# tatary/ramses

Hardware: AMD Instinct MI355X
Metric: cell-updates/s (Godunov sweep), uniform Sedov3D (higher is better)
Workload: dtype f64

## Files before the change

ramses_amd/csrc/hydro_sweep.hip:

```cpp
#include <hip/hip_runtime.h>

#include <type_traits>

#include "difmag_core.hpp"
#include "hydro_core.hpp"
#include "sweep_args.hpp"

namespace ramses_amd {

#ifdef RAMSES_AMD_FAST
#define SWEEP_NS fastmode
#else
#define SWEEP_NS strictmode
#endif

namespace SWEEP_NS {

constexpr int BX = 64;
#ifndef TILE_SWEEP_BY
#define TILE_SWEEP_BY 12
#endif

template <int BY, int NV>
struct Plane {
  double v[NV][BY][BX];
};

template <int ST, int BY, int NV, bool MASK, bool GRAV, int NX = 0, bool DUTY = false, bool R3 = false, int DPN = 0>
struct Lds {
  static constexpr int NF = NV + NX;
  static constexpr int RING = (ST == 3 || R3) ? 3 : 2;
#ifndef SWEEP_PARK_PLAIN
#ifdef RAMSES_AMD_FAST
#define SWEEP_PARK_PLAIN 1
#else
#define SWEEP_PARK_PLAIN 0
#endif
#endif
  static constexpr bool PARK = MASK || ((GRAV || SWEEP_PARK_PLAIN) && BY == 12);
  static constexpr int MR = PARK ? BY - 2 : BY;
  static constexpr int M0 = PARK ? 1 : 0;
  static constexpr size_t q_off = 0;
  static constexpr size_t m_off = q_off + RING * sizeof(Plane<BY, NV>);
  static constexpr size_t park_off = m_off + 2 * sizeof(Plane<MR, NF>);
  static constexpr size_t duty_off = park_off + (PARK ? sizeof(double) * 2 * NF * (BY - 4) * BX : 0);
  static constexpr size_t mask_off = duty_off + (DUTY ? sizeof(double) * 2 * NF * BX : 0);
  static constexpr size_t sloc_off = mask_off + (MASK ? 3 * BY * BX : 0);
  static constexpr size_t dpark_off = sloc_off + (MASK ? 4 * BY * BX : 0);
  static constexpr size_t bytes = dpark_off + sizeof(double) * DPN * (BY - 4) * BX;
};
template <int RS, int NV>
constexpr int dif_parked() { return (NV == 5 && RS == RIEMANN_EXACT) ? 2 * NV + 2 : ((NV == 6) ? NV + 2 : 0); }

__device__ __forceinline__ double wave_shr1(double v) {
  int lo = __double2loint(v), hi = __double2hiint(v);
  lo = __builtin_amdgcn_update_dpp(lo, lo, 0x138, 0xf, 0xf, false);
  hi = __builtin_amdgcn_update_dpp(hi, hi, 0x138, 0xf, 0xf, false);
  return __hiloint2double(hi, lo);
}
template <bool TIED = false>
__device__ __forceinline__ double wave_shl1(double v) {
  int lo = __double2loint(v), hi = __double2hiint(v);
  lo = TIED ? __builtin_amdgcn_update_dpp(lo, lo, 0x130, 0xf, 0xf, false) : __builtin_amdgcn_update_dpp(0, lo, 0x130, 0xf, 0xf, true);
  hi = TIED ? __builtin_amdgcn_update_dpp(hi, hi, 0x130, 0xf, 0xf, false) : __builtin_amdgcn_update_dpp(0, hi, 0x130, 0xf, 0xf, true);
  return __hiloint2double(hi, lo);
}

enum { ROLE_HALO = 0, ROLE_LOW = 1, ROLE_HIGH = 2, ROLE_FULL = 3, ROLE_HALO_HI = 4, ROLE_FULL_LO = 5 };

#ifndef SWEEP_YDUTY
#define SWEEP_YDUTY 0
#endif
template <int ST, int RS, int BY, bool GRAV, int SCHEME, int NV, bool MASK, int NE = 0, bool PFIX = false>
constexpr bool y_duty() {
  return SWEEP_YDUTY && SWEEP_PARK_PLAIN && RS == RIEMANN_LLF && BY == 12 && ST != 3 && !GRAV && SCHEME == 0 && NV == 5 && !MASK && NE == 0 && !PFIX;
}
template <int BY, bool DUTY>
constexpr int yflux_wave(int f) { return !DUTY ? f : (f == 2 ? 0 : (f == BY - 2 ? BY - 1 : f)); }

#ifndef SWEEP_TRIM
#ifdef RAMSES_AMD_FAST
#define SWEEP_TRIM 1
#else
#define SWEEP_TRIM 0
#endif
#endif

#ifndef SWEEP_CYCLE_PROBE
#define SWEEP_CYCLE_PROBE 0
#endif
#if SWEEP_CYCLE_PROBE
constexpr int PROBE_BLOCKS = 8192, PROBE_ROWS = 12, PROBE_WORDS = 6;
static __device__ unsigned long long sweep_cycle_probe[PROBE_BLOCKS][PROBE_ROWS][PROBE_WORDS];
#endif

typedef unsigned int v2u32 __attribute__((ext_vector_type(2)));
constexpr unsigned BUF_RANGE = 0x7fffffffu;
constexpr unsigned BUF_OOB = 0xffffffffu;
#ifndef SWEEP_STORE_AUX
#define SWEEP_STORE_AUX 0
#endif
__device__ __forceinline__ double plane_load(const double *var_base, unsigned plane_bytes, unsigned off) {
  __amdgpu_buffer_rsrc_t r = __builtin_amdgcn_make_buffer_rsrc(const_cast<double *>(var_base), 0, BUF_RANGE, 0x00020000);
  return __builtin_bit_cast(double, __builtin_amdgcn_raw_buffer_load_b64(r, off, plane_bytes, 0));
}
__device__ __forceinline__ void plane_store(double *var_base, unsigned plane_bytes, unsigned off, double x) {
  __amdgpu_buffer_rsrc_t r = __builtin_amdgcn_make_buffer_rsrc(var_base, 0, BUF_RANGE, 0x00020000);
  __builtin_amdgcn_raw_buffer_store_b64(__builtin_bit_cast(v2u32, x), r, off, plane_bytes, SWEEP_STORE_AUX);
}

__device__ __forceinline__ int wave_shr1_i(int v) { return __builtin_amdgcn_update_dpp(v, v, 0x138, 0xf, 0xf, false); }
__device__ __forceinline__ int wave_shl1_i(int v) { return __builtin_amdgcn_update_dpp(0, v, 0x130, 0xf, 0xf, true); }
__device__ __forceinline__ int stat_load(const unsigned char *base, unsigned ncell, unsigned lane_cell, unsigned plane_cell) {
  __amdgpu_buffer_rsrc_t r = __builtin_amdgcn_make_buffer_rsrc(const_cast<unsigned char *>(base), 0, ncell, 0x00020000);
  return (int)__builtin_amdgcn_raw_buffer_load_b8(r, lane_cell, plane_cell, 0);
}
__device__ __forceinline__ int dir_load(const int *base, unsigned plane_ints, unsigned col) {
  __amdgpu_buffer_rsrc_t r = __builtin_amdgcn_make_buffer_rsrc(const_cast<int *>(base), 0, BUF_RANGE, 0x00020000);
  return (int)__builtin_amdgcn_raw_buffer_load_b32(r, col * 4u, plane_ints * 4u, 0);
}

template <int NV>
__device__ __forceinline__ void load_uold_cell(const double *uold, long pitch_var, unsigned odd_var, unsigned pb, unsigned off, double (&u)[NV]) {
#pragma unroll
  for (int n = 0; n < NV; n++) u[n] = plane_load(uold + (long)(n & ~1) * pitch_var, pb + (n & 1) * odd_var, off);
}
__device__ __forceinline__ unsigned tile_base_ym(int par, bool inB, unsigned a0, unsigned a1, unsigned b0, unsigned b1) {
  const unsigned a = par ? a1 : a0, b = par ? b1 : b0;
  return inB ? b : a;
}
template <int ST, int RS, int BY, bool GRAV, int SCHEME, int NV, int ROLE, bool MASK, int NE = 0, bool PFIX = false, bool DIFMAG = false>
__device__ __forceinline__ void sweep_march(const SweepArgs &A, unsigned char *smem_raw, const SweepPfix &X = SweepPfix(),
                                            const SweepDifmag &D = SweepDifmag()) {
  static_assert(!PFIX || (MASK && NE == 0 && SCHEME == 0), "pressure_fix: the sweep of a level in tiles, muscl");
  static_assert(!DIFMAG || (MASK && NE == 0 && SCHEME == 0 && !PFIX), "difmag: the sweep of a level in tiles, muscl, no pressure_fix");
  constexpr int NF = NV + (PFIX ? 2 : 0);
  const bool DXPOW2 = A.pow2 != 0;
  constexpr bool DUTY = y_duty<ST, RS, BY, GRAV, SCHEME, NV, MASK, NE, PFIX>();
  static_assert(DUTY || ROLE != ROLE_FULL_LO, "row 2 is a full row like the others unless the y fluxes are shared out");
  constexpr int DPN = DIFMAG ? dif_parked<RS, NV>() : 0;
  typedef Lds<ST, BY, NV, MASK, GRAV, NF - NV, DUTY, DIFMAG, DPN> L;
  double (*dpark)[BY - 4][BX] = reinterpret_cast<double (*)[BY - 4][BX]>(smem_raw + L::dpark_off);
  constexpr int RING = L::RING;
  constexpr bool PARK = L::PARK;
  constexpr int M0 = L::M0;
  Plane<BY, NV> *qring = reinterpret_cast<Plane<BY, NV> *>(smem_raw + L::q_off);
  Plane<L::MR, NF> *mring = reinterpret_cast<Plane<L::MR, NF> *>(smem_raw + L::m_off);
  double (*park)[BY - 4][BX] = reinterpret_cast<double (*)[BY - 4][BX]>(smem_raw + L::park_off);
  double (*yduty)[NF][BX] = reinterpret_cast<double (*)[NF][BX]>(smem_raw + L::duty_off);

  const int tx = threadIdx.x, ty = threadIdx.y;
  const HydroConst &P = A.P;

  const int hb = blockIdx.x;
  int bi = 0;
#pragma unroll
  for (int i = 1; i < 6; i++)
    if (i < A.nbox && hb >= A.box[i].first) bi = i;
  const SweepBox &B = A.box[bi];
  int lb = hb - B.first;
  {
    const int nxcd = 8;
    const int cnt = (bi + 1 < A.nbox ? A.box[bi + 1].first : (int)gridDim.x) - B.first;
    if (cnt % nxcd == 0) {
      const int per = cnt / nxcd;
      lb = (lb % nxcd) * per + lb / nxcd;
    }
  }
#ifndef SWEEP_TILE_YFAST
#define SWEEP_TILE_YFAST 0
#endif
#if SWEEP_TILE_YFAST
  const int tiy = B.ty0 + lb % B.nty;
  const int tix = B.tx0 + (lb / B.nty) % B.ntx;
#else
  const int tix = B.tx0 + lb % B.ntx;
  const int tiy = B.ty0 + (lb / B.ntx) % B.nty;
#endif
  const int tiz = lb / (B.ntx * B.nty);
  int x0 = tix * (BX - 4);
  int y0 = tiy * (BY - 4);
  int z0 = B.zlo + tiz * B.zchunk;
  int z1 = min(z0 + B.zchunk, B.zhi);
  if (MASK) {
    const int4 w = reinterpret_cast<const int4 *>(A.work)[hb];
    x0 = w.x; y0 = w.y; z0 = w.z; z1 = w.w;
  }

  const int xu = x0 - 2 + tx;
  const int yu = y0 - 2 + ty;
  int xi, yi;
  if (A.ng == 0) {
    xi = xu < 0 ? xu + A.nx : (xu >= A.nx ? xu - A.nx : xu);
    xi = xi >= A.nx ? xi % A.nx : xi;
    yi = yu < 0 ? yu + A.ny : (yu >= A.ny ? yu - A.ny : yu);
    yi = yi >= A.ny ? yi % A.ny : yi;
  } else {
    xi = min(max(xu, -A.ng), A.nx + A.ng - 1) + A.ng;
    yi = min(max(yu, -A.ng), A.ny + A.ng - 1) + A.ng;
  }
  const unsigned colb = (unsigned)(xi + yi * (int)A.pitch_y) * 8u;
  int tyu = 0, yis = 0, xa = 0, tA = 0, tB = 0, drow = 0;
  bool inB = false;
  unsigned *sloc = reinterpret_cast<unsigned *>(smem_raw + L::sloc_off);
  if (MASK) {
    tyu = __builtin_amdgcn_readfirstlane(ty);
    const int ys = y0 - 2 + tyu;
    yis = ys < 0 ? ys + A.ny : (ys >= A.ny ? ys - A.ny : ys);
    const int xs = x0 - 2;
    xa = xs < 0 ? xs + A.nx : xs;
    tA = xa >> 6; tB = tA + 1 < A.ntx ? tA + 1 : 0;
    inB = (xa & 63) + tx >= 64;
    drow = A.ntx * (yis >> 3);
    const int lind = (xi & 1) + 2 * (yis & 1);
    sloc[ty * BX + tx] = ((unsigned)((long)lind * A.ngd) + (unsigned)(((xi >> 1) & (TILE_OX - 1)) + TILE_OX * ((yis >> 1) & (TILE_OY - 1)))) * 8u;
  }
  const double *__restrict__ uold = A.uold;
  double *__restrict__ unew = A.unew;
  const double *__restrict__ grav = A.grav;

#ifndef SWEEP_LATE_BASE
#define SWEEP_LATE_BASE 0
#endif
  constexpr bool LATE = SWEEP_LATE_BASE && NV == 5;
#ifndef SWEEP_KEEP_PLAIN
#define SWEEP_KEEP_PLAIN 1
#endif
#ifndef SWEEP_KEEP_STRICT
#define SWEEP_KEEP_STRICT 0
#endif
#if defined(RAMSES_AMD_FAST) || SWEEP_KEEP_STRICT
#ifndef SWEEP_KEEP_LLF_ONLY
#define SWEEP_KEEP_LLF_ONLY 0
#endif
#ifndef SWEEP_KEEP_NOT_HLLC
#define SWEEP_KEEP_NOT_HLLC 1
#endif
  constexpr bool KEEP = (MASK || (SWEEP_KEEP_PLAIN && BY == 12)) && NV == 5 && !LATE && (!SWEEP_KEEP_LLF_ONLY || RS == RIEMANN_LLF) &&
                        (!SWEEP_KEEP_NOT_HLLC || RS != RIEMANN_HLLC);
#else
  constexpr bool KEEP = false;
#endif
  constexpr bool r_fxz = ROLE == ROLE_FULL || ROLE == ROLE_FULL_LO;
  constexpr bool r_trace = ROLE == ROLE_LOW || ROLE == ROLE_HIGH || r_fxz;
  constexpr bool y_give = DUTY && (ROLE == ROLE_FULL_LO || ROLE == ROLE_HIGH);
  constexpr bool y_take = DUTY && (ROLE == ROLE_HALO || ROLE == ROLE_HALO_HI);
  constexpr int DUTY_F = ROLE == ROLE_HALO ? 2 : BY - 2;
  static_assert(!DUTY || (yflux_wave<BY, DUTY>(2) == 0 && yflux_wave<BY, DUTY>(BY - 2) == BY - 1 && yflux_wave<BY, DUTY>(3) == 3),
                "the roles below implement this table");
  constexpr bool TRIM = SWEEP_TRIM != 0 && RS == RIEMANN_LLF && SCHEME == 0 && NE == 0 && !PFIX;
  const bool r_upd = r_fxz && (tx >= 2) && (tx <= BX - 3) && (xu < A.nx) && (yu < A.ny);
  const unsigned colb_upd = r_upd ? colb : BUF_OOB;

  const double dtdx = A.dt / A.dx;
  const double dtxhalf = A.dt * 0.5;

  auto plane_off = [&](int p) -> unsigned {
    int pz;
    if (A.ng == 0) { pz = p < 0 ? p + A.nz : (p >= A.nz ? p - A.nz : p); }
    else { pz = p + A.ng; }
    return (unsigned)pz * (unsigned)(A.pitch_z * 8);
  };
  auto wrap_z = [&](int p) -> int { return p < 0 ? p + A.nz : (p >= A.nz ? p - A.nz : p); };
  constexpr unsigned TILE_VOID = 0x80000000u;
  unsigned sA0 = TILE_VOID, sA1 = TILE_VOID, sB0 = TILE_VOID, sB1 = TILE_VOID;
  unsigned mA0 = TILE_VOID, mA1 = TILE_VOID, mB0 = TILE_VOID, mB1 = TILE_VOID;
  int drow_m = 0;
  if constexpr (DIFMAG) {
    const int ym = yis > 0 ? yis - 1 : A.ny - 1;
    drow_m = A.ntx * (ym >> 3);
  }
  auto tile_of_plane = [&](int p) -> int { return wrap_z(p) >> 3; };
  auto tile_set = [&](int tz) {
    typedef const int __attribute__((address_space(4))) *cdir_p;
    const cdir_p row = (cdir_p)(A.dir + (long)tz * (A.ntx * A.nty) + drow);
    const int ra = row[tA], rb = row[tB];
    const unsigned a = ra < 0 ? TILE_VOID : (unsigned)ra * 8u, b = rb < 0 ? TILE_VOID : (unsigned)rb * 8u;
    if (tz & 1) { sA1 = a; sB1 = b; } else { sA0 = a; sB0 = b; }
    if constexpr (DIFMAG) {
      const cdir_p rowm = (cdir_p)(A.dir + (long)tz * (A.ntx * A.nty) + drow_m);
      const int qa = rowm[tA], qb = rowm[tB];
      const unsigned am = qa < 0 ? TILE_VOID : (unsigned)qa * 8u, bm = qb < 0 ? TILE_VOID : (unsigned)qb * 8u;
      if (tz & 1) { mA1 = am; mB1 = bm; } else { mA0 = am; mB0 = bm; }
    }
  };
  auto zpart = [&](int p) -> unsigned {
    const int pz = wrap_z(p);
    return (unsigned)((long)(pz & 1) * 4 * A.ngd) + (unsigned)(TILE_OX * TILE_OY * ((pz >> 1) & (TILE_OZ - 1)));
  };
  auto tbp = [&](int p) -> unsigned {
    const int par = tile_of_plane(p) & 1;
    const unsigned a = par ? sA1 : sA0, b = par ? sB1 : sB0;
    return (inB ? b : a) + sloc[ty * BX + tx];
  };
  const unsigned odd_var = (unsigned)(A.pitch_var * 8);
  auto load_u = [&](int p, double (&u)[NV]) {
    const unsigned pb = MASK ? zpart(p) * 8u : plane_off(p), off = MASK ? tbp(p) : colb;
#pragma unroll
    for (int n = 0; n < NV; n++)
      u[n] = MASK ? plane_load(uold + (long)(n & ~1) * A.pitch_var, pb + (n & 1) * odd_var, off) : plane_load(uold + (long)n * A.pitch_var, pb, off);
  };
  const double *__restrict__ bsrc = A.base_uold ? uold : unew;
  auto load_base = [&](int p, double (&u)[NF]) {
    const unsigned pb = zpart(p) * 8u, off = tbp(p);
#pragma unroll
    for (int n = 0; n < NV; n++) u[n] = plane_load(bsrc + (long)(n & ~1) * A.pitch_var, pb + (n & 1) * odd_var, off);
    if constexpr (PFIX) { u[NV] = plane_load(X.divu, pb, off); u[NV + 1] = plane_load(X.enew, pb, off); }
  };
  double dif_cy = 0.0;
  double dif_c0 = 0.0, dif_c1 = 0.0;
  int ok_zlo = 0;
  int spre = 0;
  unsigned char *smask = smem_raw + L::mask_off;
  auto load_g = [&](int p, double (&g)[3]) {
    if (GRAV) {
      const unsigned pb = MASK ? zpart(p) * 8u : plane_off(p), off = MASK ? tbp(p) : colb;
#pragma unroll
      for (int d = 0; d < 3; d++) g[d] = plane_load(grav + (long)d * A.pitch_var, pb, off);
    } else {
      g[0] = g[1] = g[2] = 0.0;
    }
  };

  double qmz[NV];
  double fzlo[NF];
  double upre[NV], gpre[3];
  double rold = 0.0, sold[NV > 5 ? NV - 5 : 1];
  double ukeep[NV];
#pragma unroll
  for (int n = 0; n < NV; n++) ukeep[n] = 0.0;

  double rinv_c = 0.0;
#if SWEEP_CYCLE_PROBE
  unsigned long long pr_a = 0, pr_w = 0, pr_b = 0, pr_n = 0;
#endif

  int sa = 0, sb = 1, sc = 2;

  if (MASK) {
    const int t0 = tile_of_plane(z0 - 2), t1 = t0 + 1 < A.ntz ? t0 + 1 : 0;
    tile_set(t0);
    tile_set(t1);
    __syncthreads();
    if (r_trace) spre = stat_load(A.stat, (unsigned)A.pitch_var, tbp(z0 - 1) >> 3, zpart(z0 - 1));
  }
  {
    double u[NV], g[3], q[NV];
    load_u(z0 - 2, u); load_g(z0 - 2, g);
    ctoprim_cell<NV, GRAV, NE>(u, g, dtxhalf, P, q);
#pragma unroll
    for (int n = 0; n < NV; n++) qring[sa].v[n][ty][tx] = q[n];
    load_u(z0 - 1, u); load_g(z0 - 1, g);
    if (KEEP) {
#pragma unroll
      for (int n = 0; n < NV; n++) ukeep[n] = u[n];
    }
    if constexpr (TRIM && r_trace) ctoprim_cell<NV, GRAV, NE>(u, g, dtxhalf, P, q, &rinv_c);
    else ctoprim_cell<NV, GRAV, NE>(u, g, dtxhalf, P, q);
#pragma unroll
    for (int n = 0; n < NV; n++) qring[sb].v[n][ty][tx] = q[n];
    load_u(z0, upre); load_g(z0, gpre);
#pragma unroll
    for (int n = 0; n < NV; n++) qmz[n] = 1.0;
#pragma unroll
    for (int n = 0; n < NF; n++) fzlo[n] = 0.0;
  }
  __builtin_amdgcn_s_waitcnt(0x0f70);
  __syncthreads();

  const int txm = tx - 1, txp = tx + 1;
  const int tym = ty - 1, typ = ty + 1;

  double partx[NF];
  double fyown[NF];
  double rnew = 0.0, snew[NV > 5 ? NV - 5 : 1];
  double bcar[NV];
#pragma unroll
  for (int n = 0; n < NV; n++) bcar[n] = 0.0;
#pragma unroll
  for (int n = 0; n < NF; n++) { partx[n] = 0.0; fyown[n] = 0.0; }
  if (PARK && r_fxz) {
#pragma unroll
    for (int n = 0; n < 2 * NF; n++) park[n][ty - 2][tx] = 0.0;
  }
  if constexpr (DUTY && ROLE == ROLE_FULL_LO) {
#pragma unroll
    for (int n = 0; n < NF; n++) yduty[0][n][tx] = yduty[1][n][tx] = 0.0;
  }
  if constexpr (DPN > 0 && (ROLE == ROLE_FULL || ROLE == ROLE_FULL_LO)) {
#pragma unroll
    for (int n = 0; n < DPN; n++) dpark[n][ty - 2][tx] = n < NV + 2 ? 0.0 : 1.0;
  }

  for (int c = z0 - 1; c <= z1; c++) {
    Plane<L::MR, NF> &M = mring[c & 1];
    Plane<L::MR, NF> &Mprev = mring[(c & 1) ^ 1];
#if SWEEP_CYCLE_PROBE
    const unsigned long long pr_t0 = __builtin_readcyclecounter();
#endif
    double qc[NV];
    double rinv_n = 0.0;
    if constexpr (TRIM && r_trace) ctoprim_cell<NV, GRAV, NE>(upre, gpre, dtxhalf, P, qc, &rinv_n);
    else ctoprim_cell<NV, GRAV, NE>(upre, gpre, dtxhalf, P, qc);
    if (RING == 3 || !r_trace) {
#pragma unroll
      for (int n = 0; n < NV; n++) qring[RING == 3 ? sc : sa].v[n][ty][tx] = qc[n];
    }
    double ucur[NF];
    if (r_fxz && !LATE && !DIFMAG) {
      if (KEEP && (!MASK || A.base_uold)) {
#pragma unroll
        for (int n = 0; n < NV; n++) ucur[n] = ukeep[n];
      } else if constexpr (MASK) load_base(c, ucur);
      else load_u(c, ucur);
    }
    if (KEEP && r_fxz) {
#pragma unroll
      for (int n = 0; n < NV; n++) ukeep[n] = upre[n];
    }
    int okc = 0, ok_ym = 0;
    if (MASK && r_trace) {
      okc = spre;
      smask[((c + 3) % 3 * BY + ty) * BX + tx] = (unsigned char)okc;
    }

    double qpy[NV], dz[NF], px[NF];
    if (ST == 3) __syncthreads();
    if constexpr (r_trace) {
      const Plane<BY, NV> &qs = qring[sb];
      const Plane<BY, NV> &qprev = qring[sa];
      double qb[NV], dq[3][NV];
      if (ST == 3) {
        const Plane<BY, NV> &qnext = qring[sc];
        const int xs[3] = {txm, tx, txp}, ys[3] = {tym, ty, typ};
#pragma unroll
        for (int n = 0; n < NV; n++) {
          double nb[27], d3[3];
#pragma unroll
          for (int dj = 0; dj < 3; dj++)
#pragma unroll
            for (int di = 0; di < 3; di++) {
              nb[di + 3 * dj] = qprev.v[n][ys[dj]][xs[di]];
              nb[di + 3 * dj + 9] = qs.v[n][ys[dj]][xs[di]];
              nb[di + 3 * dj + 18] = qnext.v[n][ys[dj]][xs[di]];
            }
          qb[n] = nb[13];
          slope3_var(nb, d3);
          dq[0][n] = d3[0]; dq[1][n] = d3[1]; dq[2][n] = d3[2];
        }
      } else if (ST == 4 || ST == 5 || ST == 6) {
#pragma unroll
        for (int n = 0; n < NV; n++) qb[n] = qs.v[n][ty][tx];
        const double dc0 = qb[1] * A.dt / A.dx, dc1 = qb[2] * A.dt / A.dx, dc2 = qb[3] * A.dt / A.dx;
#pragma unroll
        for (int n = 0; n < NV; n++) {
          dq[0][n] = slope1_1d<ST>(qs.v[n][ty][txm], qb[n], qs.v[n][ty][txp], dc0, n);
          dq[1][n] = slope1_1d<ST>(qs.v[n][tym][tx], qb[n], qs.v[n][typ][tx], dc1, n);
          dq[2][n] = slope1_1d<ST>(qprev.v[n][ty][tx], qb[n], qc[n], dc2, n);
        }
      } else {
#pragma unroll
        for (int n = 0; n < NV; n++) {
          qb[n] = qs.v[n][ty][tx];
          dq[0][n] = slope1<ST>(qs.v[n][ty][txm], qb[n], qs.v[n][ty][txp], P);
          dq[1][n] = slope1<ST>(qs.v[n][tym][tx], qb[n], qs.v[n][typ][tx], P);
          dq[2][n] = slope1<ST>(qprev.v[n][ty][tx], qb[n], qc[n], P);
        }
      }
      if (RING == 2) {
#pragma unroll
        for (int n = 0; n < NV; n++) qring[sa].v[n][ty][tx] = qc[n];
      }
      double qm[3][NV], qp[3][NV];
      if (SCHEME == 0) {
        if constexpr (TRIM) trace3d_cell<NV, NE, r_fxz>(qb, dq, dtdx, dtdx, dtdx, P, qm, qp, &rinv_c);
        else trace3d_cell<NV, NE, r_fxz>(qb, dq, dtdx, dtdx, dtdx, P, qm, qp);
      } else {
        const double cc = ctoprim_sound(qb[0], qb[4], P);
        tracexyz_cell<NV>(qb, dq, cc, dtdx, dtdx, dtdx, P, qm, qp);
      }
#pragma unroll
      for (int n = 0; n < NV; n++) M.v[n][ty - M0][tx] = (DUTY && ROLE == ROLE_HIGH) ? qp[1][n] : qm[1][n];
#pragma unroll
      for (int n = 0; n < NV; n++) qpy[n] = qp[1][n];
      if constexpr (DUTY && ROLE == ROLE_FULL_LO) {
#pragma unroll
        for (int n = 0; n < NV; n++) yduty[c & 1][n][tx] = qp[1][n];
      }
      if constexpr (r_fxz) {
        double qL[NV], fx[NF], fz[NF];
#pragma unroll
        for (int n = 0; n < NV; n++) qL[n] = wave_shr1(qm[0][n]);
        if constexpr (PFIX) {
          double f[NV], t[2];
          scaled_interface_flux_tmp<RS, NV, 0>(qL, qp[0], P, A.dt, A.dx, A.rdx, DXPOW2, f, t);
#pragma unroll
          for (int n = 0; n < NV; n++) fx[n] = f[n];
          fx[NV] = t[0]; fx[NV + 1] = t[1];
          scaled_interface_flux_tmp<RS, NV, 2>(qmz, qp[2], P, A.dt, A.dx, A.rdx, DXPOW2, f, t);
#pragma unroll
          for (int n = 0; n < NV; n++) fz[n] = f[n];
          fz[NV] = t[0]; fz[NV + 1] = t[1];
        } else {
        scaled_interface_flux<RS, NV, 0, !MASK, NE, TRIM>(qL, qp[0], P, A.dt, A.dx, A.rdx, dtdx, DXPOW2, fx);
        if constexpr (DPN > NV + 2) {
#pragma unroll
          for (int n = 0; n < NV; n++) qmz[n] = dpark[NV + 2 + n][ty - 2][tx];
        }
        scaled_interface_flux<RS, NV, 2, !MASK, NE, TRIM>(qmz, qp[2], P, A.dt, A.dx, A.rdx, dtdx, DXPOW2, fz);
        }
        if (MASK && !DIFMAG) {
          const int s_xm = wave_shr1_i(okc);
          const bool zx = ((okc | s_xm) & CELL_REFINED) != 0, zz = ((okc | ok_zlo) & CELL_REFINED) != 0;
#pragma unroll
          for (int n = 0; n < NF; n++) { fx[n] = zx ? 0.0 : fx[n]; fz[n] = zz ? 0.0 : fz[n]; }
        }
        double fxh[NF];
#pragma unroll
        for (int n = 0; n < NV; n++) qmz[n] = qm[2][n];
        if constexpr (DPN > NV + 2) {
#pragma unroll
          for (int n = 0; n < NV; n++) dpark[NV + 2 + n][ty - 2][tx] = qm[2][n];
        }
        if constexpr (DIFMAG) {
#pragma unroll
          for (int n = 0; n < NF; n++) { px[n] = fx[n]; dz[n] = fz[n]; }
        } else {
#pragma unroll
        for (int n = 0; n < NF; n++) {
          dz[n] = fzlo[n] - fz[n];
          fzlo[n] = fz[n];
          fxh[n] = wave_shl1(fx[n]);
          px[n] = LATE ? (fx[n] - fxh[n]) : ucur[n] + (fx[n] - fxh[n]);
        }
        }
        if (NV > 5 + NE && !MASK) {
          rnew = ucur[0];
#pragma unroll
          for (int n = 5 + NE; n < NV; n++) snew[n - 5] = ucur[n];
        }
      }
    }
    __builtin_amdgcn_sched_barrier(0);
    if constexpr (DIFMAG && (r_fxz || ROLE == ROLE_HIGH)) {
      static_assert(!KEEP && !LATE && PARK, "difmag borrows ukeep, bcar and partx");
      double (&dif_u)[NV] = ukeep, (&dif_uym)[NV] = bcar, (&dif_uzm)[NV] = partx;
      load_uold_cell<NV>(uold, A.pitch_var, odd_var, zpart(c) * 8u, tbp(c), dif_u);
      if constexpr (!r_fxz)
        load_uold_cell<NV>(uold, A.pitch_var, odd_var, zpart(c) * 8u,
                           tile_base_ym(tile_of_plane(c) & 1, inB, mA0, mA1, mB0, mB1) + sloc[(ty - 1) * BX + tx], dif_uym);
      if constexpr (r_fxz) {
        load_uold_cell<NV>(uold, A.pitch_var, odd_var, zpart(c - 1) * 8u, tbp(c - 1), dif_uzm);
        load_base(c, ucur);
      }
    }
    {
      const int pn = min(c + 2, z1 + 1);
      if (MASK) {
        const int lp = wrap_z(pn) & 7;
        const int tn = tile_of_plane(pn) + 1 < A.ntz ? tile_of_plane(pn) + 1 : 0;
        if (lp == 4) tile_set(tn);
      }
      load_u(pn, upre); load_g(pn, gpre);
      if (MASK && r_trace) { const int ps = min(c + 1, z1 + 1); spre = stat_load(A.stat, (unsigned)A.pitch_var, tbp(ps) >> 3, zpart(ps)); }
    }
    __builtin_amdgcn_sched_barrier(0);
#if SWEEP_CYCLE_PROBE
    const unsigned long long pr_t1 = __builtin_readcyclecounter();
#endif
    __syncthreads();
#if SWEEP_CYCLE_PROBE
    const unsigned long long pr_t2 = __builtin_readcyclecounter();
#endif

    if constexpr (DIFMAG && (r_fxz || ROLE == ROLE_HIGH)) {
      double (&dif_u)[NV] = ukeep, (&dif_uym)[NV] = bcar, (&dif_uzm)[NV] = partx;
      const Plane<BY, NV> &q0 = qring[sb], &q1 = qring[sc];
      constexpr int NR = r_fxz ? 3 : 2;
      const double fdiv = 0.25 / A.dx;
      double dsum[3][2];
#pragma unroll
      for (int d = 0; d < 3; d++) {
        double vo[2][NR], vl[2][NR];
#pragma unroll
        for (int r = 0; r < NR; r++) {
          vo[0][r] = q0.v[1 + d][tym + r][tx];
          vo[1][r] = q1.v[1 + d][tym + r][tx];
          vl[0][r] = wave_shr1(vo[0][r]);
          vl[1][r] = wave_shr1(vo[1][r]);
        }
#pragma unroll
        for (int r0 = 0; r0 < NR - 1; r0++) {
          double v[2][2][2];
#pragma unroll
          for (int dk = 0; dk < 2; dk++)
#pragma unroll
            for (int dj = 0; dj < 2; dj++) { v[dk][dj][0] = vl[dk][r0 + dj]; v[dk][dj][1] = vo[dk][r0 + dj]; }
          dsum[d][r0] = d == 0 ? difmag::cmpdivu_ux(v, fdiv) : (d == 1 ? difmag::cmpdivu_vy(v, fdiv) : difmag::cmpdivu_wz(v, fdiv));
        }
        if (NR == 2) dsum[d][1] = 0.0;
      }
      const double dn[2] = {dsum[0][0] + dsum[1][0] + dsum[2][0], dsum[0][1] + dsum[1][1] + dsum[2][1]};
      if constexpr (DPN > 0 && r_fxz) {
        dif_c0 = dpark[NV][ty - 2][tx]; dif_c1 = dpark[NV + 1][ty - 2][tx];
#pragma unroll
        for (int n = 0; n < NV; n++) fzlo[n] = dpark[n][ty - 2][tx];
      }
      const double c0x = wave_shl1<true>(dif_c0), n0x = wave_shl1<true>(dn[0]);
      dif_cy = difmag::consup_coef(D.difmag, difmag::consup_div1_y(dif_c0, c0x, dn[0], n0x));
      if constexpr (r_fxz) {
        const double c1x = wave_shl1<true>(dif_c1);
        const double cx = difmag::consup_coef(D.difmag, difmag::consup_div1_x(dif_c0, dif_c1, dn[0], dn[1]));
        const double cz = difmag::consup_coef(D.difmag, difmag::consup_div1_z(dif_c0, c0x, dif_c1, c1x));
        const int s_xm = wave_shr1_i(okc);
        const bool zx = ((okc | s_xm) & CELL_REFINED) != 0, zz = ((okc | ok_zlo) & CELL_REFINED) != 0;
#pragma unroll
        for (int n = 0; n < NV; n++) {
          const double fxd = difmag::consup_term(px[n], A.dt, cx, dif_u[n], wave_shr1(dif_u[n]));
          const double fzd = difmag::consup_term(dz[n], A.dt, cz, dif_u[n], dif_uzm[n]);
          const double fxn = zx ? 0.0 : fxd, fzn = zz ? 0.0 : fzd;
          dz[n] = fzlo[n] - fzn;
          fzlo[n] = fzn;
          px[n] = ucur[n] + (fxn - wave_shl1<true>(fxn));
        }
      }
      dif_c0 = dn[0]; dif_c1 = dn[1];
      if constexpr (DPN > 0 && r_fxz) {
        dpark[NV][ty - 2][tx] = dn[0]; dpark[NV + 1][ty - 2][tx] = dn[1];
#pragma unroll
        for (int n = 0; n < NV; n++) dpark[n][ty - 2][tx] = fzlo[n];
      }
      if constexpr (r_fxz)
        load_uold_cell<NV>(uold, A.pitch_var, odd_var, zpart(c) * 8u,
                           tile_base_ym(tile_of_plane(c) & 1, inB, mA0, mA1, mB0, mB1) + sloc[(ty - 1) * BX + tx], dif_uym);
    }
    double fy[NF];
    if constexpr (y_take) {
      double qL[NV], qR[NV];
#pragma unroll
      for (int n = 0; n < NV; n++) {
        qL[n] = M.v[n][DUTY_F - 1 - M0][tx];
        qR[n] = ROLE == ROLE_HALO ? yduty[c & 1][n][tx] : M.v[n][DUTY_F - M0][tx];
      }
      scaled_interface_flux<RS, NV, 1, !MASK, NE, TRIM>(qL, qR, P, A.dt, A.dx, A.rdx, dtdx, DXPOW2, fy);
#pragma unroll
      for (int n = 0; n < NF; n++) {
        if (ROLE == ROLE_HALO) yduty[c & 1][n][tx] = fy[n];
        else M.v[n][DUTY_F - 1 - M0][tx] = fy[n];
      }
    }
    if constexpr ((r_fxz || ROLE == ROLE_HIGH) && !y_give) {
      double qL[NV];
#pragma unroll
      for (int n = 0; n < NV; n++) qL[n] = M.v[n][tym - M0][tx];
      if constexpr (PFIX) {
        double f[NV], t[2];
        scaled_interface_flux_tmp<RS, NV, 1>(qL, qpy, P, A.dt, A.dx, A.rdx, DXPOW2, f, t);
#pragma unroll
        for (int n = 0; n < NV; n++) fy[n] = f[n];
        fy[NV] = t[0]; fy[NV + 1] = t[1];
      } else {
      scaled_interface_flux<RS, NV, 1, !MASK, NE, TRIM>(qL, qpy, P, A.dt, A.dx, A.rdx, dtdx, DXPOW2, fy);
      }
      if constexpr (DIFMAG) {
        double (&dif_u)[NV] = ukeep, (&dif_uym)[NV] = bcar;
#pragma unroll
        for (int n = 0; n < NV; n++) fy[n] = difmag::consup_term(fy[n], A.dt, dif_cy, dif_u[n], dif_uym[n]);
      }
      if (MASK) {
        ok_ym = smask[((c + 3) % 3 * BY + tym) * BX + tx];
        const bool zy = ((okc | ok_ym) & CELL_REFINED) != 0;
#pragma unroll
        for (int n = 0; n < NF; n++) fy[n] = zy ? 0.0 : fy[n];
      }
#pragma unroll
      for (int n = 0; n < NF; n++) M.v[n][tym - M0][tx] = fy[n];
    }
    if constexpr (r_fxz) {
      double un[NF], fyh[NF];
#pragma unroll
      for (int n = 0; n < NF; n++) {
        fyh[n] = Mprev.v[n][ty - M0][tx];
        const double pxn = PARK ? park[n][ty - 2][tx] : partx[n];
        const double fyn = y_give ? yduty[(c & 1) ^ 1][n][tx] : (PARK ? park[NF + n][ty - 2][tx] : fyown[n]);
        const double part = (LATE ? bcar[n < NV ? n : 0] + pxn : pxn) + (fyn - fyh[n]);
        un[n] = part + dz[n];
      }
      if (NV > 5 + NE && !MASK) {
        if (rold < P.smallr && un[0] > rold) {
#pragma unroll
          for (int n = 5 + NE; n < NV; n++) un[n] = sold[n - 5] * dmaxd(un[0], P.smallr) / P.smallr;
        } else if (un[0] < P.smallr && rold > un[0]) {
#pragma unroll
          for (int n = 5 + NE; n < NV; n++) un[n] = sold[n - 5] * P.smallr / dmaxd(rold, P.smallr);
        }
        rold = rnew;
#pragma unroll
        for (int n = 5 + NE; n < NV; n++) sold[n - 5] = snew[n - 5];
      }
#pragma unroll
      for (int n = 0; n < NF; n++) {
        if (PARK) { park[n][ty - 2][tx] = px[n]; if (!y_give) park[NF + n][ty - 2][tx] = fy[n]; }
        else { partx[n] = px[n]; fyown[n] = fy[n]; }
      }
      {
        const unsigned pb = MASK ? zpart(c - 1) * 8u : plane_off(c - 1);
        const unsigned so = (c >= z0 + 1) ? (MASK ? ((r_upd && (ok_zlo & CELL_OWNED)) ? tbp(c - 1) : BUF_OOB) : colb_upd) : BUF_OOB;
#pragma unroll
        for (int n = 0; n < NV; n++) {
          if (MASK) plane_store(unew + (long)(n & ~1) * A.pitch_var, pb + (n & 1) * odd_var, so, un[n]);
          else plane_store(unew + (long)n * A.pitch_var, pb, so, un[n]);
        }
        if constexpr (PFIX) { plane_store(X.divu, pb, so, un[NV]); plane_store(X.enew, pb, so, un[NV + 1]); }
      }
      if constexpr (LATE) { if (MASK) load_base(c, bcar); else load_u(c, bcar); }
    }
    if (RING == 3) { const int t = sa; sa = sb; sb = sc; sc = t; }
    else { const int t = sa; sa = sb; sb = t; }
    if (MASK) ok_zlo = okc;
    if (TRIM) rinv_c = rinv_n;
#if SWEEP_CYCLE_PROBE
    pr_a += pr_t1 - pr_t0; pr_w += pr_t2 - pr_t1; pr_b += __builtin_readcyclecounter() - pr_t2; pr_n += 1;
#endif
  }
#if SWEEP_CYCLE_PROBE
  if (tx == 0 && blockIdx.x < PROBE_BLOCKS && ty < PROBE_ROWS) {
    unsigned long long *o = sweep_cycle_probe[blockIdx.x][ty];
    o[0] = pr_a; o[1] = pr_w; o[2] = pr_b; o[3] = pr_n; o[4] = (unsigned long long)ty;
    o[5] = (unsigned long long)__builtin_amdgcn_s_getreg((31 << 11) | 4);
  }
#endif
}

template <int ST, int RS, int BY, bool GRAV, int SCHEME, int NV, bool MASK = false>
__global__ __launch_bounds__(BX *BY) void godunov_sweep_kernel(SweepArgs A) {
  extern __shared__ __attribute__((aligned(16))) unsigned char smem_raw[];
  const int ty = threadIdx.y;
  if (ty >= 2 && ty <= BY - 3) __builtin_amdgcn_s_setprio(3);
  if (ty == 0) sweep_march<ST, RS, BY, GRAV, SCHEME, NV, ROLE_HALO, MASK>(A, smem_raw);
  else if (ty == BY - 1) sweep_march<ST, RS, BY, GRAV, SCHEME, NV, ROLE_HALO_HI, MASK>(A, smem_raw);
  else if (ty == 1) sweep_march<ST, RS, BY, GRAV, SCHEME, NV, ROLE_LOW, MASK>(A, smem_raw);
  else if (ty == BY - 2) sweep_march<ST, RS, BY, GRAV, SCHEME, NV, ROLE_HIGH, MASK>(A, smem_raw);
  else {
    if constexpr (y_duty<ST, RS, BY, GRAV, SCHEME, NV, MASK>()) {
      if (ty == 2) { sweep_march<ST, RS, BY, GRAV, SCHEME, NV, ROLE_FULL_LO, MASK>(A, smem_raw); return; }
    }
    sweep_march<ST, RS, BY, GRAV, SCHEME, NV, ROLE_FULL, MASK>(A, smem_raw);
  }
}

#ifndef RAMSES_AMD_FAST
template <int ST, int NV>
struct PfixRows {
  static constexpr int BY = (ST == 3 && NV == 7) ? 6 : 8;
};
template <int ST, int RS, int BY, bool GRAV, int NV>
__global__ __launch_bounds__(BX *BY) void godunov_sweep_pfix_kernel(SweepArgs A, SweepPfix X) {
  extern __shared__ __attribute__((aligned(16))) unsigned char smem_raw[];
  static_assert(Lds<ST, BY, NV, true, GRAV, 2>::bytes <= 160 * 1024, "the pressure_fix sweep fits one workgroup's LDS");
  const int ty = threadIdx.y;
  if (ty >= 2 && ty <= BY - 3) __builtin_amdgcn_s_setprio(3);
  if (ty == 0) sweep_march<ST, RS, BY, GRAV, 0, NV, ROLE_HALO, true, 0, true>(A, smem_raw, X);
  else if (ty == BY - 1) sweep_march<ST, RS, BY, GRAV, 0, NV, ROLE_HALO_HI, true, 0, true>(A, smem_raw, X);
  else if (ty == 1) sweep_march<ST, RS, BY, GRAV, 0, NV, ROLE_LOW, true, 0, true>(A, smem_raw, X);
  else if (ty == BY - 2) sweep_march<ST, RS, BY, GRAV, 0, NV, ROLE_HIGH, true, 0, true>(A, smem_raw, X);
  else sweep_march<ST, RS, BY, GRAV, 0, NV, ROLE_FULL, true, 0, true>(A, smem_raw, X);
}
#endif

#ifndef RAMSES_AMD_FAST
template <int ST, int RS, int BY, bool GRAV, int NV>
__global__ __launch_bounds__(BX *BY) void godunov_sweep_difmag_kernel(SweepArgs A, SweepDifmag D) {
  extern __shared__ __attribute__((aligned(16))) unsigned char smem_raw[];
  static_assert(Lds<ST, BY, NV, true, GRAV, 0, false, true, dif_parked<RS, NV>()>::bytes <= 160 * 1024, "the difmag sweep fits one workgroup's LDS");
  const int ty = threadIdx.y;
  if (ty >= 2 && ty <= BY - 3) __builtin_amdgcn_s_setprio(3);
  if (ty == 0) sweep_march<ST, RS, BY, GRAV, 0, NV, ROLE_HALO, true, 0, false, true>(A, smem_raw, SweepPfix(), D);
  else if (ty == BY - 1) sweep_march<ST, RS, BY, GRAV, 0, NV, ROLE_HALO_HI, true, 0, false, true>(A, smem_raw, SweepPfix(), D);
  else if (ty == 1) sweep_march<ST, RS, BY, GRAV, 0, NV, ROLE_LOW, true, 0, false, true>(A, smem_raw, SweepPfix(), D);
  else if (ty == BY - 2) sweep_march<ST, RS, BY, GRAV, 0, NV, ROLE_HIGH, true, 0, false, true>(A, smem_raw, SweepPfix(), D);
  else sweep_march<ST, RS, BY, GRAV, 0, NV, ROLE_FULL, true, 0, false, true>(A, smem_raw, SweepPfix(), D);
}
#endif

template <int ST, int RS, int NV, int NE>
__global__ __launch_bounds__(BX * 8) void godunov_sweep_nener_kernel(SweepArgs A) {
  extern __shared__ __attribute__((aligned(16))) unsigned char smem_raw[];
  constexpr int BY = 8;
  const int ty = threadIdx.y;
  if (ty >= 2 && ty <= BY - 3) __builtin_amdgcn_s_setprio(3);
  if (ty == 0) sweep_march<ST, RS, BY, false, 0, NV, ROLE_HALO, false, NE>(A, smem_raw);
  else if (ty == BY - 1) sweep_march<ST, RS, BY, false, 0, NV, ROLE_HALO_HI, false, NE>(A, smem_raw);
  else if (ty == 1) sweep_march<ST, RS, BY, false, 0, NV, ROLE_LOW, false, NE>(A, smem_raw);
  else if (ty == BY - 2) sweep_march<ST, RS, BY, false, 0, NV, ROLE_HIGH, false, NE>(A, smem_raw);
  else sweep_march<ST, RS, BY, false, 0, NV, ROLE_FULL, false, NE>(A, smem_raw);
}

template <int ST, int RS, int NE>
struct ScalarGroup {
  static constexpr int RING = (ST == 3) ? 3 : 2;
  static constexpr int NH = 5 + NE;
  static constexpr int G = (ST == 3 ? 8 : 10) - (RS == RIEMANN_EXACT ? 2 : 0) - NH;
  static constexpr int NV = NH + G;
  static constexpr size_t m_off = RING * sizeof(Plane<8, NV>);
  static constexpr size_t bytes = m_off + 2 * sizeof(Plane<8, NV>);
  static_assert(G >= 1 && bytes <= 160 * 1024, "the scalar pass fits one workgroup's LDS");
};

template <int ST, int RS, bool GRAV, int NE, int ROLE>
__device__ __forceinline__ void scalar_march(const SweepArgs &A, int s0, int nlive, unsigned char *smem_raw) {
  typedef ScalarGroup<ST, RS, NE> SG;
  constexpr int BY = 8, RING = SG::RING, NH = SG::NH, G = SG::G, NV = SG::NV;
  const bool DXPOW2 = A.pow2 != 0;
  Plane<BY, NV> *qring = reinterpret_cast<Plane<BY, NV> *>(smem_raw);
  Plane<BY, NV> *mring = reinterpret_cast<Plane<BY, NV> *>(smem_raw + SG::m_off);
  const int tx = threadIdx.x, ty = threadIdx.y;
  const HydroConst &P = A.P;

  const int hb = blockIdx.x;
  int bi = 0;
#pragma unroll
  for (int i = 1; i < 6; i++)
    if (i < A.nbox && hb >= A.box[i].first) bi = i;
  const SweepBox &B = A.box[bi];
  int lb = hb - B.first;
  {
    const int nxcd = 8;
    const int cnt = (bi + 1 < A.nbox ? A.box[bi + 1].first : (int)gridDim.x) - B.first;
    if (cnt % nxcd == 0) {
      const int per = cnt / nxcd;
      lb = (lb % nxcd) * per + lb / nxcd;
    }
  }
  const int tix = B.tx0 + lb % B.ntx;
  const int tiy = B.ty0 + (lb / B.ntx) % B.nty;
  const int tiz = lb / (B.ntx * B.nty);
  const int x0 = tix * (BX - 4), y0 = tiy * (BY - 4);
  const int z0 = B.zlo + tiz * B.zchunk;
  const int z1 = min(z0 + B.zchunk, B.zhi);
  const int xu = x0 - 2 + tx, yu = y0 - 2 + ty;
  int xi, yi;
  if (A.ng == 0) {
    xi = xu < 0 ? xu + A.nx : (xu >= A.nx ? xu - A.nx : xu);
    xi = xi >= A.nx ? xi % A.nx : xi;
    yi = yu < 0 ? yu + A.ny : (yu >= A.ny ? yu - A.ny : yu);
    yi = yi >= A.ny ? yi % A.ny : yi;
  } else {
    xi = min(max(xu, -A.ng), A.nx + A.ng - 1) + A.ng;
    yi = min(max(yu, -A.ng), A.ny + A.ng - 1) + A.ng;
  }
  const unsigned colb = (unsigned)(xi + yi * (int)A.pitch_y) * 8u;
  const double *__restrict__ uold = A.uold;
  double *__restrict__ unew = A.unew;
  const double *__restrict__ grav = A.grav;

  constexpr bool r_trace = ROLE == ROLE_LOW || ROLE == ROLE_HIGH || ROLE == ROLE_FULL;
  constexpr bool r_fxz = ROLE == ROLE_FULL;
  const bool r_upd = r_fxz && (tx >= 2) && (tx <= BX - 3) && (xu < A.nx) && (yu < A.ny);
  const unsigned colb_upd = r_upd ? colb : BUF_OOB;
  const double dtdx = A.dt / A.dx;
  const double dtxhalf = A.dt * 0.5;

  auto plane_off = [&](int p) -> unsigned {
    int pz;
    if (A.ng == 0) { pz = p < 0 ? p + A.nz : (p >= A.nz ? p - A.nz : p); }
    else { pz = p + A.ng; }
    return (unsigned)pz * (unsigned)(A.pitch_z * 8);
  };
  auto var_of = [&](int n) -> long { return n < NH ? n : s0 + min(n - NH, nlive - 1); };
  auto load_u = [&](int p, double (&u)[NV]) {
    const unsigned pb = plane_off(p);
#pragma unroll
    for (int n = 0; n < NV; n++) u[n] = plane_load(uold + var_of(n) * A.pitch_var, pb, colb);
  };
  auto load_g = [&](int p, double (&g)[3]) {
    if (GRAV) {
      const unsigned pb = plane_off(p);
#pragma unroll
      for (int d = 0; d < 3; d++) g[d] = plane_load(grav + (long)d * A.pitch_var, pb, colb);
    } else {
      g[0] = g[1] = g[2] = 0.0;
    }
  };

  double qmz[NV];
  double fzlo[G];
  double upre[NV], gpre[3];
  double rold = 0.0, sold[G];
  double rnew = 0.0;
  double partx[G], fyown[G], dz[G], px[G], fy[G];
  int sa = 0, sb = 1, sc = 2;
  {
    double u[NV], g[3], q[NV];
    load_u(z0 - 2, u); load_g(z0 - 2, g);
    ctoprim_cell<NV, GRAV, NE>(u, g, dtxhalf, P, q);
#pragma unroll
    for (int n = 0; n < NV; n++) qring[sa].v[n][ty][tx] = q[n];
    load_u(z0 - 1, u); load_g(z0 - 1, g);
    ctoprim_cell<NV, GRAV, NE>(u, g, dtxhalf, P, q);
#pragma unroll
    for (int n = 0; n < NV; n++) qring[sb].v[n][ty][tx] = q[n];
    load_u(z0, upre); load_g(z0, gpre);
#pragma unroll
    for (int n = 0; n < NV; n++) qmz[n] = 1.0;
#pragma unroll
    for (int j = 0; j < G; j++) { fzlo[j] = 0.0; sold[j] = 0.0; partx[j] = 0.0; fyown[j] = 0.0; dz[j] = 0.0; px[j] = 0.0; }
  }
  __builtin_amdgcn_s_waitcnt(0x0f70);
  __syncthreads();
  const int txm = tx - 1, txp = tx + 1;
  const int tym = ty - 1, typ = ty + 1;

  for (int c = z0 - 1; c <= z1; c++) {
    Plane<BY, NV> &M = mring[c & 1];
    Plane<BY, NV> &Mprev = mring[(c & 1) ^ 1];
    double qc[NV];
    ctoprim_cell<NV, GRAV, NE>(upre, gpre, dtxhalf, P, qc);
    if (RING == 3 || !r_trace) {
#pragma unroll
      for (int n = 0; n < NV; n++) qring[RING == 3 ? sc : sa].v[n][ty][tx] = qc[n];
    }
    double rnew_m = 0.0;
    double ucur[G];
    if (r_fxz) {
      const unsigned pc = plane_off(c);
      rnew = plane_load(uold, pc, colb);
#pragma unroll
      for (int j = 0; j < G; j++) ucur[j] = plane_load(uold + var_of(NH + j) * A.pitch_var, pc, colb);
      rnew_m = plane_load(unew, plane_off(c - 1), colb);
    }
    double qpy[NV];
    if (ST == 3) __syncthreads();
    if constexpr (r_trace) {
      const Plane<BY, NV> &qs = qring[sb];
      const Plane<BY, NV> &qprev = qring[sa];
      double qb[NV], dq[3][NV];
      if (ST == 3) {
        const Plane<BY, NV> &qnext = qring[sc];
        const int xs[3] = {txm, tx, txp}, ys[3] = {tym, ty, typ};
#pragma unroll
        for (int n = 0; n < NV; n++) {
          double nb[27], d3[3];
#pragma unroll
          for (int dj = 0; dj < 3; dj++)
#pragma unroll
            for (int di = 0; di < 3; di++) {
              nb[di + 3 * dj] = qprev.v[n][ys[dj]][xs[di]];
              nb[di + 3 * dj + 9] = qs.v[n][ys[dj]][xs[di]];
              nb[di + 3 * dj + 18] = qnext.v[n][ys[dj]][xs[di]];
            }
          qb[n] = nb[13];
          slope3_var(nb, d3);
          dq[0][n] = d3[0]; dq[1][n] = d3[1]; dq[2][n] = d3[2];
        }
      } else {
#pragma unroll
        for (int n = 0; n < NV; n++) {
          qb[n] = qs.v[n][ty][tx];
          dq[0][n] = slope1<ST>(qs.v[n][ty][txm], qb[n], qs.v[n][ty][txp], P);
          dq[1][n] = slope1<ST>(qs.v[n][tym][tx], qb[n], qs.v[n][typ][tx], P);
          dq[2][n] = slope1<ST>(qprev.v[n][ty][tx], qb[n], qc[n], P);
        }
      }
      if (RING == 2) {
#pragma unroll
        for (int n = 0; n < NV; n++) qring[sa].v[n][ty][tx] = qc[n];
      }
      double qm[3][NV], qp[3][NV];
      trace3d_cell<NV, NE>(qb, dq, dtdx, dtdx, dtdx, P, qm, qp);
#pragma unroll
      for (int n = 0; n < NV; n++) M.v[n][ty][tx] = qm[1][n];
#pragma unroll
      for (int n = 0; n < NV; n++) qpy[n] = qp[1][n];
      if constexpr (r_fxz) {
        double qL[NV], fx[NV], fz[NV];
#pragma unroll
        for (int n = 0; n < NV; n++) qL[n] = wave_shr1(qm[0][n]);
        scaled_interface_flux<RS, NV, 0, true, NE>(qL, qp[0], P, A.dt, A.dx, A.rdx, dtdx, DXPOW2, fx);
        scaled_interface_flux<RS, NV, 2, true, NE>(qmz, qp[2], P, A.dt, A.dx, A.rdx, dtdx, DXPOW2, fz);
#pragma unroll
        for (int n = 0; n < NV; n++) qmz[n] = qm[2][n];
#pragma unroll
        for (int j = 0; j < G; j++) {
          dz[j] = fzlo[j] - fz[NH + j];
          fzlo[j] = fz[NH + j];
          px[j] = ucur[j] + (fx[NH + j] - wave_shl1(fx[NH + j]));
        }
      }
    }
    __builtin_amdgcn_sched_barrier(0);
    {
      const int pn = min(c + 2, z1 + 1);
      load_u(pn, upre); load_g(pn, gpre);
    }
    __builtin_amdgcn_sched_barrier(0);
    __syncthreads();

    if constexpr (ROLE == ROLE_FULL || ROLE == ROLE_HIGH) {
      double qL[NV], f[NV];
#pragma unroll
      for (int n = 0; n < NV; n++) qL[n] = M.v[n][tym][tx];
      scaled_interface_flux<RS, NV, 1, true, NE>(qL, qpy, P, A.dt, A.dx, A.rdx, dtdx, DXPOW2, f);
#pragma unroll
      for (int j = 0; j < G; j++) { fy[j] = f[NH + j]; M.v[NH + j][tym][tx] = fy[j]; }
    }
    if constexpr (r_fxz) {
      double un[G];
#pragma unroll
      for (int j = 0; j < G; j++) un[j] = (partx[j] + (fyown[j] - Mprev.v[NH + j][ty][tx])) + dz[j];
      if (rold < P.smallr && rnew_m > rold) {
#pragma unroll
        for (int j = 0; j < G; j++) un[j] = sold[j] * dmaxd(rnew_m, P.smallr) / P.smallr;
      } else if (rnew_m < P.smallr && rold > rnew_m) {
#pragma unroll
        for (int j = 0; j < G; j++) un[j] = sold[j] * P.smallr / dmaxd(rold, P.smallr);
      }
      rold = rnew;
#pragma unroll
      for (int j = 0; j < G; j++) { sold[j] = ucur[j]; partx[j] = px[j]; fyown[j] = fy[j]; }
      const unsigned pb = plane_off(c - 1);
      const unsigned so = (c >= z0 + 1) ? colb_upd : BUF_OOB;
#pragma unroll
      for (int j = 0; j < G; j++)
        if (j < nlive) plane_store(unew + var_of(NH + j) * A.pitch_var, pb, so, un[j]);
    }
    if (RING == 3) { const int t = sa; sa = sb; sb = sc; sc = t; }
    else { const int t = sa; sa = sb; sb = t; }
  }
}

template <int ST, int RS, bool GRAV, int NE>
__global__ __launch_bounds__(BX * 8) void godunov_scalar_kernel(SweepArgs A, int s0, int nlive) {
// ... 600 lines not shown
```

Baseline: 46.21 billion.

## Issue next-plane loads early and carry z-plane offsets incrementally

```diff
diff --git a/ramses_amd/csrc/hydro_sweep.hip b/ramses_amd/csrc/hydro_sweep.hip
--- a/ramses_amd/csrc/hydro_sweep.hip
+++ b/ramses_amd/csrc/hydro_sweep.hip
@@ -90,7 +90,7 @@
 #define SWEEP_CYCLE_PROBE 0
 #endif
 #if SWEEP_CYCLE_PROBE
-constexpr int PROBE_BLOCKS = 8192, PROBE_ROWS = 12, PROBE_WORDS = 6;
+constexpr int PROBE_BLOCKS = 8192, PROBE_ROWS = 12, PROBE_WORDS = 8;
 static __device__ unsigned long long sweep_cycle_probe[PROBE_BLOCKS][PROBE_ROWS][PROBE_WORDS];
 #endif
 
@@ -249,6 +249,25 @@
   static_assert(!DUTY || (yflux_wave<BY, DUTY>(2) == 0 && yflux_wave<BY, DUTY>(BY - 2) == BY - 1 && yflux_wave<BY, DUTY>(3) == 3),
                 "the roles below implement this table");
   constexpr bool TRIM = SWEEP_TRIM != 0 && RS == RIEMANN_LLF && SCHEME == 0 && NE == 0 && !PFIX;
+#ifndef SWEEP_EARLY_PREFETCH
+#define SWEEP_EARLY_PREFETCH 1
+#endif
+#ifndef SWEEP_EARLY_GRAV
+#define SWEEP_EARLY_GRAV 0
+#endif
+#ifndef SWEEP_EARLY_STRICT
+#define SWEEP_EARLY_STRICT 0
+#endif
+#if defined(RAMSES_AMD_FAST) || SWEEP_EARLY_STRICT
+  constexpr bool EARLY = SWEEP_EARLY_PREFETCH != 0 && !MASK && BY == 12 && RS == RIEMANN_LLF && SCHEME == 0 && NV == 5 && NE == 0 && !PFIX &&
+                         (!GRAV || SWEEP_EARLY_GRAV);
+#else
+  constexpr bool EARLY = false;
+#endif
+#ifndef SWEEP_PLANE_CARRY
+#define SWEEP_PLANE_CARRY 1
+#endif
+  constexpr bool CARRY = SWEEP_PLANE_CARRY != 0 && !MASK && BY == 12 && RS == RIEMANN_LLF && SCHEME == 0 && NV == 5 && NE == 0 && !PFIX;
   const bool r_upd = r_fxz && (tx >= 2) && (tx <= BX - 3) && (xu < A.nx) && (yu < A.ny);
   const unsigned colb_upd = r_upd ? colb : BUF_OOB;
 
@@ -260,6 +279,11 @@
     if (A.ng == 0) { pz = p < 0 ? p + A.nz : (p >= A.nz ? p - A.nz : p); }
     else { pz = p + A.ng; }
     return (unsigned)pz * (unsigned)(A.pitch_z * 8);
+  };
+  const unsigned zpitch = (unsigned)(A.pitch_z * 8);
+  const unsigned zwrap = A.ng == 0 ? (unsigned)A.nz * zpitch : 0u;
+  auto plane_next = [&](unsigned off, int p1) -> unsigned {
+    return off + zpitch - (((p1 == 0) | (p1 == A.nz)) ? zwrap : 0u);
   };
   auto wrap_z = [&](int p) -> int { return p < 0 ? p + A.nz : (p >= A.nz ? p - A.nz : p); };
   constexpr unsigned TILE_VOID = 0x80000000u;
@@ -322,6 +346,19 @@
     }
   };
 
+  auto load_u_at = [&](unsigned pb, double (&u)[NV]) {
+#pragma unroll
+    for (int n = 0; n < NV; n++) u[n] = plane_load(uold + (long)n * A.pitch_var, pb, colb);
+  };
+  auto load_g_at = [&](unsigned pb, double (&g)[3]) {
+    if (GRAV) {
+#pragma unroll
+      for (int d = 0; d < 3; d++) g[d] = plane_load(grav + (long)d * A.pitch_var, pb, colb);
+    } else {
+      g[0] = g[1] = g[2] = 0.0;
+    }
+  };
+
   double qmz[NV];
   double fzlo[NF];
   double upre[NV], gpre[3];
@@ -332,7 +369,7 @@
 
   double rinv_c = 0.0;
 #if SWEEP_CYCLE_PROBE
-  unsigned long long pr_a = 0, pr_w = 0, pr_b = 0, pr_n = 0;
+  unsigned long long pr_a = 0, pr_w = 0, pr_b = 0, pr_n = 0, pr_b2 = 0, pr_b3 = 0;
 #endif
 
   int sa = 0, sb = 1, sc = 2;
@@ -391,6 +428,17 @@
 #pragma unroll
     for (int n = 0; n < DPN; n++) dpark[n][ty - 2][tx] = n < NV + 2 ? 0.0 : 1.0;
   }
+  unsigned zo_m = 0, zo_c = 0, zo_p = 0, zo_n = 0;
+  if constexpr (CARRY) { zo_m = plane_off(z0 - 2); zo_c = plane_off(z0 - 1); zo_p = plane_off(z0); }
+  auto request_next = [&](int c) {
+    if constexpr (CARRY) {
+      const unsigned pb = c == z1 ? zo_p : zo_n;
+      load_u_at(pb, upre); load_g_at(pb, gpre);
+    } else {
+      const int pn = min(c + 2, z1 + 1);
+      load_u(pn, upre); load_g(pn, gpre);
+    }
+  };
 
   for (int c = z0 - 1; c <= z1; c++) {
     Plane<L::MR, NF> &M = mring[c & 1];
@@ -398,6 +446,7 @@
 #if SWEEP_CYCLE_PROBE
     const unsigned long long pr_t0 = __builtin_readcyclecounter();
 #endif
+    if constexpr (CARRY) zo_n = plane_next(zo_p, c + 2);
     double qc[NV];
     double rinv_n = 0.0;
     if constexpr (TRIM && r_trace) ctoprim_cell<NV, GRAV, NE>(upre, gpre, dtxhalf, P, qc, &rinv_n);
@@ -412,11 +461,17 @@
 #pragma unroll
         for (int n = 0; n < NV; n++) ucur[n] = ukeep[n];
       } else if constexpr (MASK) load_base(c, ucur);
+      else if constexpr (CARRY) load_u_at(zo_c, ucur);
       else load_u(c, ucur);
     }
     if (KEEP && r_fxz) {
 #pragma unroll
       for (int n = 0; n < NV; n++) ukeep[n] = upre[n];
+    }
+    if constexpr (EARLY) {
+      __builtin_amdgcn_sched_barrier(0);
+      request_next(c);
+      __builtin_amdgcn_sched_barrier(0);
     }
     int okc = 0, ok_ym = 0;
     if (MASK && r_trace) {
@@ -554,7 +609,9 @@
         load_base(c, ucur);
       }
     }
-    {
+    if constexpr (CARRY || EARLY) {
+      if constexpr (!EARLY) request_next(c);
+    } else {
       const int pn = min(c + 2, z1 + 1);
       if (MASK) {
         const int lp = wrap_z(pn) & 7;
@@ -676,6 +733,13 @@
 #pragma unroll
       for (int n = 0; n < NF; n++) M.v[n][tym - M0][tx] = fy[n];
     }
+#if SWEEP_CYCLE_PROBE
+    __builtin_amdgcn_sched_barrier(0);
+    const unsigned long long pr_t3 = __builtin_readcyclecounter();
+    __builtin_amdgcn_s_waitcnt(0x0f70);
+    const unsigned long long pr_t4 = __builtin_readcyclecounter();
+    __builtin_amdgcn_sched_barrier(0);
+#endif
     if constexpr (r_fxz) {
       double un[NF], fyh[NF];
 #pragma unroll
@@ -704,7 +768,7 @@
         else { partx[n] = px[n]; fyown[n] = fy[n]; }
       }
       {
-        const unsigned pb = MASK ? zpart(c - 1) * 8u : plane_off(c - 1);
+        const unsigned pb = MASK ? zpart(c - 1) * 8u : (CARRY ? zo_m : plane_off(c - 1));
         const unsigned so = (c >= z0 + 1) ? (MASK ? ((r_upd && (ok_zlo & CELL_OWNED)) ? tbp(c - 1) : BUF_OOB) : colb_upd) : BUF_OOB;
 #pragma unroll
         for (int n = 0; n < NV; n++) {
@@ -713,14 +777,18 @@
         }
         if constexpr (PFIX) { plane_store(X.divu, pb, so, un[NV]); plane_store(X.enew, pb, so, un[NV + 1]); }
       }
-      if constexpr (LATE) { if (MASK) load_base(c, bcar); else load_u(c, bcar); }
+      if constexpr (LATE) { if (MASK) load_base(c, bcar); else if constexpr (CARRY) load_u_at(zo_c, bcar); else load_u(c, bcar); }
     }
     if (RING == 3) { const int t = sa; sa = sb; sb = sc; sc = t; }
     else { const int t = sa; sa = sb; sb = t; }
     if (MASK) ok_zlo = okc;
     if (TRIM) rinv_c = rinv_n;
+    if constexpr (CARRY) { zo_m = zo_c; zo_c = zo_p; zo_p = zo_n; }
 #if SWEEP_CYCLE_PROBE
-    pr_a += pr_t1 - pr_t0; pr_w += pr_t2 - pr_t1; pr_b += __builtin_readcyclecounter() - pr_t2; pr_n += 1;
+    {
+      const unsigned long long pr_t5 = __builtin_readcyclecounter();
+      pr_a += pr_t1 - pr_t0; pr_w += pr_t2 - pr_t1; pr_b += pr_t5 - pr_t2; pr_b2 += pr_t4 - pr_t3; pr_b3 += pr_t5 - pr_t4; pr_n += 1;
+    }
 #endif
   }
 #if SWEEP_CYCLE_PROBE
@@ -728,6 +796,7 @@
     unsigned long long *o = sweep_cycle_probe[blockIdx.x][ty];
     o[0] = pr_a; o[1] = pr_w; o[2] = pr_b; o[3] = pr_n; o[4] = (unsigned long long)ty;
     o[5] = (unsigned long long)__builtin_amdgcn_s_getreg((31 << 11) | 4);
+    o[6] = pr_b2; o[7] = pr_b3;
   }
 #endif
 }
```

Measured after the change: 42.40 billion. 0.918x the previous value.
